# n00b001/neuro-genetic-pong-self-play

Measured on AMD Instinct MI355X. Metric: env-steps/sec (GA evaluation loop, self-play) + generations/sec at pop=65536 per GPU, higher is better.
Workload: dtype f32 hidden + certified f64 argmax; genomes f64

## Files before the change

neuro-genetic-pong-self-play_amd/csrc/pg_cascade.hpp:

```cpp
#pragma once

#include <hip/hip_runtime.h>
#include <stdint.h>

#include "pg_device.hpp"
#include "pg_eval.hpp"
#include "pg_f64math.h"

namespace pg {

#ifndef PG_SLOW_INLINE
#define PG_SLOW_INLINE __forceinline__
#endif
#ifndef PG_LOAD_BATCH
#define PG_LOAD_BATCH 2
#endif
#ifndef PG_RES_WAVES
#define PG_RES_WAVES 0
#endif
#if PG_RES_WAVES > 0
#define PG_RES_BOUNDS __launch_bounds__(256, PG_RES_WAVES)
#else
#define PG_RES_BOUNDS __launch_bounds__(256)
#endif
// ... 234 lines not shown
  n.e = v[D + P * O * 2 + O];
  n.ct = make_cert(n.e);
}

template <int U, int O>
__device__ __forceinline__ void load_rec(NetP<U, O> &n, const float *__restrict__ r) {
  constexpr int P = NetP<U, O>::P;
  constexpr int F = rec_floats<U, O>();
  const float4 *s = reinterpret_cast<const float4 *>(r);
  float v[F];
#pragma unroll
  for (int q = 0; q < F / 4; ++q) {
    const float4 x = s[q];
    v[4 * q] = x.x;
    v[4 * q + 1] = x.y;
    v[4 * q + 2] = x.z;
    v[4 * q + 3] = x.w;
  }
#pragma unroll
  for (int p = 0; p < P; ++p)
#pragma unroll
    for (int i = 0; i < 7; ++i) n.w1[p][i] = float2v{v[(p * 7 + i) * 2], v[(p * 7 + i) * 2 + 1]};
#pragma unroll
  for (int p = 0; p < P; ++p)
#pragma unroll
    for (int o = 0; o < O; ++o) n.w2[p][o] = float2v{v[P * 14 + (p * O + o) * 2], v[P * 14 + (p * O + o) * 2 + 1]};
#pragma unroll
  for (int o = 0; o < O; ++o) n.c[o] = v[P * 14 + P * O * 2 + o];
  n.e = v[P * 14 + P * O * 2 + O];
  n.ct = make_cert(n.e);
}

template <int U, int O, bool kBiasIn = false>
__device__ __forceinline__ void partial_pk(const NetP<U, O> &n, const int k[6], float acc[O]) {
  constexpr int P = NetP<U, O>::P;
  float2v kx[6];
#pragma unroll
  for (int i = 0; i < 6; ++i) {
    const float f = (float)k[i];
    kx[i] = float2v{f, f};
  }
  float2v a2[O];
#pragma unroll
  for (int o = 0; o < O; ++o) a2[o] = kBiasIn ? float2v{n.c[o], n.c[o]} : float2v{0.f, 0.f};
#pragma unroll
  for (int p = 0; p < P; p += 2) {
    constexpr int kStep = 2;
    const bool two = p + 1 < P;
    float2v a = n.w1[p][6], b = two ? n.w1[p + 1][6] : float2v{0.f, 0.f};
#pragma unroll
    for (int i = 0; i < 6; ++i) {
      a = __builtin_elementwise_fma(n.w1[p][i], kx[i], a);
      if (two) b = __builtin_elementwise_fma(n.w1[p + 1][i], kx[i], b);
    }
    const float2v qa = float2v{__builtin_amdgcn_exp2f(a.x), __builtin_amdgcn_exp2f(a.y)} + 1.0f;
    const float2v qb = float2v{__builtin_amdgcn_exp2f(b.x), __builtin_amdgcn_exp2f(b.y)} + 1.0f;
    const float2v sa = float2v{__builtin_amdgcn_rcpf(qa.x), __builtin_amdgcn_rcpf(qa.y)};
    const float2v sb = float2v{__builtin_amdgcn_rcpf(qb.x), __builtin_amdgcn_rcpf(qb.y)};
#pragma unroll
    for (int o = 0; o < O; ++o) {
      a2[o] = __builtin_elementwise_fma(n.w2[p][o], sa, a2[o]);
      if (two) a2[o] = __builtin_elementwise_fma(n.w2[p + 1][o], sb, a2[o]);
    }
    (void)kStep;
  }
#pragma unroll
  for (int o = 0; o < O; ++o) acc[o] = a2[o].x + a2[o].y;
}

template <int HL, int U, int O>
__device__ __forceinline__ float frame_bound_wave(const float *__restrict__ rec, const int k[6], int lane64) {
  constexpr int P = NetP<U, O>::P;
  constexpr int F = rec_floats<U, O>();
  constexpr float kOR = (float)out_roundings<HL, U>();
  float acc[O];
#pragma unroll
  for (int o = 0; o < O; ++o) acc[o] = 0.f;
#pragma unroll 1
  for (int t = lane64; t < HL * 2 * P; t += 64) {
    const int hl = t % HL, u = t / HL, p = u >> 1, h = u & 1;
    const float *r = rec + hl * F;
    float w[7];
#pragma unroll
    for (int i = 0; i < 7; ++i) w[i] = r[(p * 7 + i) * 2 + h];
    float w2[O];
#pragma unroll
    for (int o = 0; o < O; ++o) w2[o] = r[P * 14 + (p * O + o) * 2 + h];
    float a = w[6], rr = fabsf(w[6]), ws = fabsf(w[6]);
#pragma unroll
    for (int i = 0; i < 6; ++i) {
      a = fmaf(w[i], (float)k[i], a);
      rr = fmaf(fabsf(w[i]), (float)k[i], rr);
      ws += fabsf(w[i]);
    }
    const float da = (rr + ws * (320.f * 9.5367431640625e-7f)) * (11.f * kU);
    const float sl = fminf(0.25f, __builtin_amdgcn_exp2f(2.f * da - fabsf(a)));
    const float s = __builtin_amdgcn_rcpf(__builtin_amdgcn_exp2f(a) + 1.0f);
    const float ds = sl * da * 0.6931471805599453f + s * ((5.f + kOR) * kU) + 7.8886090522101181e-31f;
#pragma unroll
    for (int o = 0; o < O; ++o) acc[o] = fmaf(fabsf(w2[o]), ds, acc[o]);
// ... 28 lines not shown
      top1 = gt ? z[o] : top1;
    }
  }
  const float tw = __builtin_amdgcn_exp2f(__builtin_fmaf(top1, 1.4426950408889634f, c.ee));
  const int uns_res = (top1 - top2 > c.e2 + tw && top1 > c.lowz) ? w : -1;
  return top1 >= c.tlo ? sat_res : uns_res;
}

template <int O>
__device__ __forceinline__ int certify_c8(const float z[O], const Cert &c) {
  if constexpr (O == 3) {
    const float top1 = fmaxf(fmaxf(z[0], z[1]), z[2]);
    const float top2 = __builtin_amdgcn_fmed3f(z[0], z[1], z[2]);
    const int wc = z[0] == top1 ? -6 : (z[1] == top1 ? 6 : 0);
    const float tw = __builtin_amdgcn_exp2f(__builtin_fmaf(top1, 1.4426950408889634f, c.ee));
#ifndef PG_CERT_FULL_SAT
    const bool ok = ((top2 < c.tlo) & (top1 > c.thi)) | ((top1 < c.tlo) & (top1 - top2 > c.e2 + tw) & (top1 > c.lowz));
    return ok ? wc : -1;
#else
    const bool m0 = z[0] >= c.tlo, m1 = z[1] >= c.tlo;
    const int fc = m0 ? -6 : (m1 ? 6 : 0);
    const float zf = m0 ? z[0] : (m1 ? z[1] : z[2]);
    const int sat_res = zf > c.thi ? fc : -1;
    const int uns_res = (top1 - top2 > c.e2 + tw && top1 > c.lowz) ? wc : -1;
    return top1 >= c.tlo ? sat_res : uns_res;
#endif
  } else {
    const int idx = certify_c<O>(z, c);
    return idx < 0 ? -1 : index_to_move(idx);
  }
}

template <int O>
__device__ __forceinline__ int tight_gap_move(const float z[O], float e, const Cert &c) {
  float top1, top2;
  int w;
  if constexpr (O == 3) {
    top1 = fmaxf(fmaxf(z[0], z[1]), z[2]);
    top2 = __builtin_amdgcn_fmed3f(z[0], z[1], z[2]);
    w = z[0] == top1 ? 0 : (z[1] == top1 ? 1 : 2);
  } else {
    top1 = z[0];
    top2 = -3.0e38f;
    w = 0;
#pragma unroll
    for (int o = 1; o < O; ++o) {
      const bool gt = z[o] > top1;
      top2 = gt ? top1 : fmaxf(top2, z[o]);
      w = gt ? o : w;
      top1 = gt ? z[o] : top1;
    }
  }
  const float tw = __builtin_amdgcn_exp2f(__builtin_fmaf(top1, 1.4426950408889634f, -51.985645f)) +
                   4.4408921e-16f;
  const bool ok = (top2 - e >= 22.2f) & (top1 < c.tlo) & (top1 - top2 > (2.f * e + tw) * 1.000001f);
  return ok ? index_to_move(w) : -1;
}

template <int O>
__device__ __forceinline__ int certify(const float z[O], float e) {
  constexpr float kTlo = 36.7367f, kThi = 36.7369f;
  constexpr float kLowZ = -708.0f;
  const float tlo = kTlo - e, thi = kThi + e;
  int sat_res = z[O - 1] > thi ? O - 1 : -1;
#pragma unroll
  for (int o = O - 2; o >= 0; --o) sat_res = z[o] > thi ? o : (z[o] >= tlo ? -1 : sat_res);
// ... 405 lines not shown
```

neuro-genetic-pong-self-play_amd/csrc/pg_device.hpp:

```cpp
#pragma once

#include <hip/hip_runtime.h>
#include <stdint.h>

#include "pg_f64math.h"

namespace pg {

#define PG_ANY(c) __builtin_expect(__builtin_amdgcn_ballot_w64(c) != 0, 0)

constexpr int kFieldW = 160;
constexpr int kFieldH = 160;
constexpr int kPaddleH = 16;
constexpr int kPaddleW = 4;
constexpr int kLeftPaddleX = 16;
constexpr int kRightPaddleX = 140;
constexpr int kBallH = 4;
constexpr int kBallW = 2;
constexpr int kPaddleYMin = -8;
constexpr int kPaddleYMax = 152;
constexpr int kPaddleSpeed = 3;
constexpr int kCpuSpeed = 2;
constexpr int kServeDelay = 30;
constexpr int kBallVx0 = 2;
// ... 152 lines not shown
  k = (k << 8) | (uint64_t)((s.rpy + 8) & 255);
  k = (k << 2) | (uint64_t)(act_r & 3);
  k = (k << 2) | (uint64_t)(act_l & 3);
  return k;
}
#ifndef PG_RALLY_START
#define PG_RALLY_START 256
#endif
#ifndef PG_RALLY_STRIDE
#define PG_RALLY_STRIDE 4
#endif
constexpr int kRallyStart = PG_RALLY_START;
constexpr int kRallyStride = PG_RALLY_STRIDE;
#ifndef PG_RALLY_SPAN0
#define PG_RALLY_SPAN0 64
#endif
constexpr int kRallyHits = 8;
static_assert(kRallyHits <= 8, "rally_key caps hits at 8");
constexpr int kRallySpan0 = PG_RALLY_SPAN0;

__device__ inline int paddle_c2(int py) {
  const int lo = py < 0 ? 0 : py;
  const int hi = py + kPaddleH - 1 > kFieldH - 1 ? kFieldH - 1 : py + kPaddleH - 1;
  return lo + hi;
}

__device__ inline int clamp_action(int c2, int code) {
  return c2 < 32 ? 2 : (c2 > 2 * (kFieldH - 16) ? 1 : code);
}
__device__ inline int clamp_move(int c2, int move) {
  static_assert(kPaddleSpeed == 3, "doubled moves of 6");
  return c2 < 32 ? 6 : (c2 > 2 * (kFieldH - 16) ? -6 : move);
}
__device__ inline int move_code(int move) { return move < 0 ? 1 : (move > 0 ? 2 : 0); }

__device__ inline int hardcoded(int by2, int me2) { return by2 < me2 ? 1 : (by2 > me2 ? 2 : 0); }
__device__ inline int hardcoded_move(int by2, int me2) { return by2 < me2 ? -6 : (by2 > me2 ? 6 : 0); }

__device__ inline int index_to_code(int idx) {
  return (int)__builtin_amdgcn_ubfe(9u, 2u * (unsigned)idx, 2u);
}
__device__ inline int index_to_move(int idx) {
  return (int)__builtin_amdgcn_sbfe(0x0006FA, 8u * (unsigned)idx, 8u);
}

struct PongK {
  int bx2, by2, vx2, vy2, vis, timer, dir, hits, point, lc2, rc2, s1, s2, one_player;
  uint64_t seed;
  static_assert(kBallH == 4 && kPaddleH == 16 && kBallW == 2, "the doubled-unit constants below");
  static constexpr int kC2Reset = 2 * 72 + kPaddleH - 1;

  __device__ void reset(uint64_t s, int one_p) {
    bx2 = 2 * 79 + kBallW - 1; by2 = 2 * 78 + kBallH - 1; vx2 = 0; vy2 = 0; vis = 0; timer = kServeDelay;
    dir = 1; hits = 0; point = 0; lc2 = kC2Reset; rc2 = kC2Reset; s1 = 0; s2 = 0; one_player = one_p; seed = s;
  }
  __device__ bool done() const { return s1 >= kDoneScore || s2 >= kDoneScore; }

  __device__ static int c2_clip(int c2) { return paddle_c2((c2 - (kPaddleH - 1)) >> 1); }
  __device__ static int drift2(int c2, int h) {
    const int down = c2 <= 31 ? min((37 - c2) / 6, h) : 0;
    const int up = c2 >= 289 ? min((c2 - 283) / 6, h) : 0;
    return c2 + 2 * kPaddleSpeed * (down - up);
  }

  template <class ServeOf>
  __device__ int step(int right_move, int left_move, ServeOf serve_of, bool any_one_player) {
    int ev = kStepFly;
    rc2 += right_move;
    int nl = lc2 + left_move;
    if (__builtin_expect(any_one_player, 0)) {
      const int cpu_dy = vis ? ((by2 < lc2 - 4) ? -1 : ((by2 > lc2 + 4) ? 1 : 0)) : 0;
      const int moved = lc2 + 2 * kCpuSpeed * cpu_dy;
      constexpr int lo = 2 * kPaddleYMin + kPaddleH - 1, hi = 2 * kPaddleYMax + kPaddleH - 1;
      nl = one_player ? (moved < lo ? lo : (moved > hi ? hi : moved)) : nl;
    }
    lc2 = nl;

    constexpr int top2 = kBallH - 1;
    constexpr int bot2 = 2 * (kFieldH - kBallH) + kBallH - 1;
    constexpr int lface = kLeftPaddleX + kPaddleW, rface = kRightPaddleX;
    constexpr int left2 = 2 * (lface - 1) + kBallW - 1;
    constexpr int right2 = 2 * (rface - kBallW + 1) + kBallW - 1;
    const bool play = vis != 0;
    const int nx2 = bx2 + vx2;
    int ny2 = by2 + vy2;
    const bool wall_top = ny2 < top2, wall_bot = ny2 > bot2;
    ny2 = wall_top ? 2 * top2 - ny2 : (wall_bot ? 2 * bot2 - ny2 : ny2);
    vy2 = (wall_top || wall_bot) ? -vy2 : vy2;
    const bool to_left = play && nx2 <= left2;
    const bool to_right = play && nx2 >= right2;
    bx2 = nx2;
    by2 = ny2;
    if (PG_ANY(to_left || to_right || !play)) {
    if (to_left || to_right) {
      const int d = ny2 - (to_left ? lc2 : rc2);
      if (d >= -18 && d <= 18) {
        hits += 1;
        const int mag = min(kBallVx0 + (hits >> 2), kBallVxMax);
        const int q = (abs(d) * 43) >> 8;
        bx2 = to_left ? 2 * lface + kBallW - 1 : 2 * (rface - kBallW) + kBallW - 1;
        vx2 = to_left ? 2 * mag : -2 * mag;
        vy2 = d < 0 ? -2 * q : 2 * q;
        ev = hits >= kRallyHits ? kStepRally : kStepBounce;
      } else {
        s2 += to_left ? 1 : 0;
        s1 += to_right ? 1 : 0;
        dir = to_left ? -1 : 1;
        timer = kServeDelay;
        vis = 0;
        ev = kStepPoint;
      }
    }
    if (!play) {
      timer = timer > 0 ? timer - 1 : 0;
      if (timer == 0 && !done()) {
        const uint32_t e = serve_of(point);
        bx2 = 2 * 79 + kBallW - 1;
        by2 = 2 * (int)(e & 255u) + kBallH - 1;
        vy2 = 2 * ((int)(e >> 8) - 2);
        vx2 = 2 * dir * kBallVx0;
        hits = 0;
        vis = 1;
        point += 1;
      }
    }
    }
    return ev;
  }

  __device__ uint64_t key(int act_r, int act_l) const {
    Pong s;
    s.bx = (bx2 - (kBallW - 1)) >> 1;
    s.by = (by2 - (kBallH - 1)) >> 1;
    s.vx = vx2 >> 1;
    s.vy = vy2 >> 1;
    s.vis = vis;
    s.timer = timer;
    s.dir = dir;
    s.hits = hits;
    s.point = point;
    s.lpy = (lc2 - (kPaddleH - 1)) >> 1;
    s.rpy = (rc2 - (kPaddleH - 1)) >> 1;
    return rally_key(s, act_r, act_l);
  }
};

template <int CTRL>
__device__ __forceinline__ float dpp_mov(float v) {
  return __int_as_float(__builtin_amdgcn_update_dpp(0, __float_as_int(v), CTRL, 0xF, 0xF, false));
}

template <int L>
__device__ __forceinline__ float group_sum(float v) {
  if constexpr (L >= 2) v += dpp_mov<0xB1>(v);
  if constexpr (L >= 4) v += dpp_mov<0x4E>(v);
  if constexpr (L >= 8) v += dpp_mov<0x141>(v);
  if constexpr (L >= 16) v += dpp_mov<0x140>(v);
  if constexpr (L >= 32) {
    const auto r = __builtin_amdgcn_permlane16_swap(__float_as_uint(v), __float_as_uint(v), false, false);
    v = __uint_as_float(r[0]) + __uint_as_float(r[1]);
  }
  if constexpr (L >= 64) {
    const auto r = __builtin_amdgcn_permlane32_swap(__float_as_uint(v), __float_as_uint(v), false, false);
    v = __uint_as_float(r[0]) + __uint_as_float(r[1]);
  }
  return v;
}

template <int L>
__device__ __forceinline__ float group_max(float v) {
  if constexpr (L >= 2) v = fmaxf(v, dpp_mov<0xB1>(v));
  if constexpr (L >= 4) v = fmaxf(v, dpp_mov<0x4E>(v));
  if constexpr (L >= 8) v = fmaxf(v, dpp_mov<0x141>(v));
  if constexpr (L >= 16) v = fmaxf(v, dpp_mov<0x140>(v));
  if constexpr (L >= 32) v = fmaxf(v, __shfl_xor(v, 16, 64));
// ... 126 lines not shown
```

neuro-genetic-pong-self-play_amd/csrc/pg_service.hpp:

```cpp
#pragma once

#include <hip/hip_runtime.h>

#include "../../include/pong_ga.h"
#include "pg_cascade.hpp"
#include "pg_device.hpp"
#include "pg_eval.hpp"
#include "pg_f64math.h"

namespace pg {

#ifndef PG_SVC_PRIO
#define PG_SVC_PRIO 3
#endif
#ifndef PG_SVC_BATCH
#define PG_SVC_BATCH 1
#endif

#ifndef PG_INLINE_SVC
#define PG_INLINE_SVC 1
#endif
#ifndef PG_INLINE_PRIO
#define PG_INLINE_PRIO 3
#endif
// ... 244 lines not shown
                         d, 0, k[q]);
              }
              d |= 256;
            } else {
              d |= 512;
            }
            if (lane64 == 0) {
              slots[sl[q]].idx = d;
              __threadfence_block();
              lds_st(&slots[sl[q]].flag, 2);
            }
          }
        }
      }
    }
    return;
  }

  const int lig = threadIdx.x & (L - 1);
  const int side = lig >= HL ? 1 : 0;
  const int hl = lig & (HL - 1);
  const int leader = lane64 & ~(L - 1);
  const int wave_slot0 = __builtin_amdgcn_readfirstlane((int)(threadIdx.x >> 6)) * (64 / L) * 2;
  const auto slot_grp = [&]() { return wave_slot0 + (fresh_lane64() / L) * 2; };
  const auto slot_me = [&]() {
    const int l = fresh_lane64();
    return wave_slot0 + (l / L) * 2 + ((l & (L - 1)) >= HL ? 1 : 0);
  };
  const WT *genomes = (const WT *)p.genomes;
  const WT *opponents = (const WT *)p.opponents;

  NetP<U, O> net;
  PongK st;
  int kind = 0, act_r = 0, act_l = 0, total = 0, fstart = 0, tend = 0, c_vis = 0, tab_off = 0;
  int sframe = 0;
#ifndef PG_NO_HIDDEN_JUMP
  constexpr bool kVisByFrames = kUntraced && !kHorizon;
#else
  constexpr bool kVisByFrames = false;
#endif
  const WT *gm = genomes;
  uint32_t slow = 0, c_fwd = 0, c_steps = 0, c_games = 0, fails = 0, plateau = 0, inwave = 0, skipped = 0, hidden = 0;

  const int games_total = active_total(p);
  int w;
  {
    int ww = 0;
    if (lig == 0) ww = (int)atomicAdd(p.work, 1u);
    w = group_broadcast<L>(ww, leader);
  }
  bool fresh = true;
  bool live = w < games_total;
  const auto park = [&]() {
    st.bx2 = 2 * 79 + kBallW - 1;
    st.by2 = 2 * 78 + kBallH - 1;
    st.vx2 = st.vy2 = 0;
    st.vis = 2;
    st.one_player = 0;
    kind = kOppNN;
    tend = 0x7fffffff;
    fstart = 0x3fffffff;
    fresh = false;
  };
  if (kInline && !live) park();
  int w_scripted = 1, w_onep = 1;
  int top = 1;
#ifdef PG_PROBE_EXTRA
  float probe_v = 0.f;
  float2v probe_p = float2v{0.f, 0.f};
  int probe_s = 0;
#endif
#ifdef PG_START_PROBE
  uint64_t probe_fresh = 0;
  const uint64_t probe_t0 = __builtin_amdgcn_s_memtime();
#endif
#ifdef PG_SERVE_STAGES
  uint64_t st_acc[24];
#pragma unroll
  for (int i = 0; i < 24; ++i) st_acc[i] = 0;
#endif
#ifdef PG_DECIDE_PROBE
  uint64_t probe_dec = 0;
  const uint64_t probe_t0 = __builtin_amdgcn_s_memtime();
#endif
#ifdef PG_TIMELINE
  uint64_t t_start = 0;
  uint32_t g_fails = 0, g_slow = 0;
#endif
#ifdef PG_PATH_PROBE
  uint32_t pp_frames = 0, pp_rally = 0, pp_face = 0, pp_fail = 0, pp_hidden = 0;
#define PG_PP(cnt, cond) \
  if (__builtin_amdgcn_ballot_w64(cond) != 0) cnt += 1
#else
#define PG_PP(cnt, cond)
#endif
  if (kInline ? __builtin_amdgcn_ballot_w64(live) != 0 : live) for (;;) {
#ifdef PG_START_PROBE
    const bool any_fresh = __builtin_amdgcn_ballot_w64(fresh) != 0;
    const uint64_t probe_f0 = __builtin_amdgcn_s_memtime();
#endif
    PG_PP(pp_frames, true);
    sframe += 1;
#ifdef PG_TIMELINE
    constexpr bool kJumps = !kHorizon;
#else
    const bool kJumps = !kHorizon && (kUntraced || p.trace == nullptr);
#endif
    if (top) {
    if (fresh) {
      const int i = w / p.n_games;
      const int g = w - i * p.n_games;
      kind = p.kind[w];
      const WT *gr = genomes + (long)genome_row(p, i) * p.gstride;
      const bool nn = side && kind == kOppNN && p.n_opponents > 0;
      const int oj = nn ? min(max(p.opp[w], 0), p.n_opponents - 1) : 0;
      gm = nn ? opponents + (long)oj * p.ostride : gr;
      const int rec = nn ? p.n_genomes + oj : i;
      load_rec<U, O>(net, p.recs + ((long)rec * HL + hl) * rec_floats<U, O>());
      const int sx = slot_me();
      if (kInline && hl == 0) slots[sx].rec = rec;
#pragma unroll
      for (int o = 0; o < O; ++o) net.c[o] = hl == 0 ? 0.5f * net.c[o] : 0.f;
      st.reset(0, kind == kOppRomCpu);
      if (kHorizon || !tabbed) st.seed = game_seed(p.seed, g);
      tab_off = g * kServeTabPoints;
      act_r = act_l = total = 0;
      c_vis = kVisByFrames ? sframe - 1 : 0;
      fstart = sframe - 1;
      tend = sframe + p.timeout_thresh;
      fresh = false;
      if (hl == 0) slots[sx].n_memo = 0;
      if (lig == 0) slots[sx].rally_at = -1;
      if (kHorizon && lig == 0) {
        const int gx = threadIdx.x / L;
        hz[gx].sum = 0.0;
        hz[gx].eps = hz[gx].s1 = hz[gx].s2 = hz[gx].zd = 0;
      }
#ifdef PG_TIMELINE
      t_start = wall_clock64();
      g_fails = g_slow = 0;
#endif
    }
#ifdef PG_START_PROBE
    if (any_fresh) probe_fresh += __builtin_amdgcn_s_memtime() - probe_f0;
#endif
#ifndef PG_NO_HIDDEN_JUMP
    {
      const bool hid = !st.vis && st.timer >= 2;
      PG_PP(pp_hidden, hid);
      if (kJumps && hid) {
        const int h = st.timer - 1;
        st.rc2 = PongK::drift2(st.rc2, h);
        if (!st.one_player) st.lc2 = PongK::drift2(st.lc2, h);
        st.timer = 1;
        act_r = clamp_move(st.rc2, 0);
        act_l = clamp_move(st.lc2, 0);
        fstart -= h;
        tend -= h;
        hidden += h;
      }
    }
#endif
    w_scripted = __builtin_amdgcn_readfirstlane(__builtin_amdgcn_ballot_w64(kind != kOppNN) != 0);
    w_onep = __builtin_amdgcn_readfirstlane(__builtin_amdgcn_ballot_w64(st.one_player != 0) != 0);
    top = 0;
    }
    const int pvis = st.vis, pbx2 = st.bx2, pby2 = st.by2;
#ifdef PG_PATH_PROBE
    const int pt_b = st.point, hits_b = st.hits;
#endif
    const int ev = st.step(act_r, act_l, [&](int pt) {
      return tabbed && pt < kServeTabPoints ? serve_tab[tab_off + pt] : Pong::serve_entry(st.seed, pt);
    }, w_onep != 0);
    PG_PP(pp_face, ev != kStepFly || st.hits != hits_b || st.point != pt_b);
    const int vis = st.vis;
    const int bx2 = st.bx2, by2 = st.by2;
    const int rc2 = st.rc2;
    int lc2 = st.lc2;
    if (__builtin_expect(w_onep, 0)) lc2 = PongK::c2_clip(st.lc2);
    int left, right;
    {
      const int lbx2 = pvis ? pbx2 : bx2, lby2 = pvis ? pby2 : by2;
      const int k[6] = {bx2, by2, lbx2, lby2, rc2, lc2};
      float acc[O], z[O];
      partial_pk<U, O, true>(net, k, acc);
#pragma unroll
      for (int o = 0; o < O; ++o) z[o] = group_sum<HL>(acc[o]);
      int code = certify_c8<O>(z, net.ct);
#ifdef PG_PROBE_EXTRA
      pg_probe_extra<PG_PROBE_EXTRA>(net.w1[0][0], net.w1[1][1], z[0], z[1], probe_v, probe_p, probe_s);
#endif
      const bool left_nn = kind == kOppNN;
      if (side && !left_nn) code = 0;
      if (vis != 1) code = 0;
#ifdef PG_ABLATE_SLOW
      if (code == -1) code = z[1] > z[0] ? 6 : -6;
#endif
      PG_PP(pp_fail, code == -1);
      if (PG_ANY(code == -1)) {
      if (code == -1) {
        fails += 1;
#ifdef PG_TIMELINE
        g_fails += 1;
#endif
#ifndef PG_NO_TIGHT
        int mv = tight_gap_move<O>(z, net.e, net.ct);
        if (mv == -1)
#else
        int mv = -1;
#endif
        {
          const int idx = plateau_f32<O>(z, net.e);
          mv = idx >= 0 ? index_to_move(idx) : -1;
        }
        inwave += mv != -1 ? 1 : 0;
        code = mv;
      }
#ifdef PG_ABLATE_SERVE
      if (code == -1) code = z[1] > z[0] ? 6 : -6;
#endif
      if (kInline && PG_ANY(code == -1)) {
        uint64_t key = 0;
        int nm = 0;
        const int sx = slot_me();
        if (code == -1) {
          key = memo_key(k);
          nm = slots[sx].n_memo;
          int hit = -1;
#pragma unroll 1
          for (int c = 0; c < kMemo && c < nm; ++c)
            if (slots[sx].memo_key[c] == key) hit = slots[sx].memo_idx[c];
          code = hit;
        }
        const int kn[6] = {side ? 320 - bx2 : bx2, by2, side ? 320 - lbx2 : lbx2, lby2, side ? lc2 : rc2,
                           side ? rc2 : lc2};
        const float my_e = net.e;
        uint64_t need = __builtin_amdgcn_ballot_w64(code == -1 && hl == 0);
        if (need) {
#ifdef PG_DECIDE_PROBE
        const uint64_t probe_d0 = __builtin_amdgcn_s_memtime();
#endif
        if constexpr (PG_INLINE_PRIO > 0) __builtin_amdgcn_s_setprio(PG_INLINE_PRIO);
#pragma unroll 1
        do {
          const int src = (int)__builtin_ctzll(need);
          need &= need - 1;
          InlineReq r;
#pragma unroll
          for (int i = 0; i < 6; ++i) r.k[i] = __builtin_amdgcn_readlane(kn[i], src);
#pragma unroll
          for (int i = 0; i < 6; ++i) r.kr[i] = __builtin_amdgcn_readlane(k[i], src);
          r.rec = p.recs + (long)__builtin_amdgcn_readlane(slots[sx].rec, src) * HL * rec_floats<U, O>();
#pragma unroll
          for (int o = O; o < 4; ++o) r.z[o] = 0.f;
#pragma unroll
          for (int o = 0; o < O; ++o) r.z[o] = __int_as_float(__builtin_amdgcn_readlane(__float_as_int(z[o]), src));
          r.e = __int_as_float(__builtin_amdgcn_readlane(__float_as_int(my_e), src));
          const uint64_t ga = (uint64_t)gm;
          const WT *g = (const WT *)(((uint64_t)__builtin_amdgcn_readlane((int)(ga >> 32), src) << 32) |
                                     (uint32_t)__builtin_amdgcn_readlane((int)(uint32_t)ga, src));
#if defined(PG_SERVE_TWICE)
          serve_inline<U, HL, O, WT>(p, g, r, lds_svc + wave * f64_lds_doubles(H, O), lane64, st_acc);
          const int ans = serve_inline<U, HL, O, WT>(p, g, r, lds_svc + wave * f64_lds_doubles(H, O), lane64, st_acc + 12);
#elif defined(PG_SERVE_STAGES)
          const int ans = serve_inline<U, HL, O, WT>(p, g, r, lds_svc + wave * f64_lds_doubles(H, O), lane64, st_acc);
#else
          const int ans = serve_inline<U, HL, O, WT>(p, g, r, lds_svc + wave * f64_lds_doubles(H, O), lane64);
#endif
          if ((lane64 & ~(HL - 1)) == src) {
            slow += (ans >> 8) & 1;
            plateau += (ans >> 9) & 1;
            inwave += ans >> 10;
            code = index_to_move(ans & 255);
            if (hl == 0) {
              const int c = nm % kMemo;
              slots[sx].memo_key[c] = key;
              slots[sx].memo_idx[c] = code;
              slots[sx].n_memo = nm + 1;
            }
          }
        } while (need);
        if constexpr (PG_INLINE_PRIO > 0) __builtin_amdgcn_s_setprio(0);
        {
#if defined(PG_RELOAD_ALL)
          load_rec<U, O>(net, p.recs + ((long)slots[sx].rec * HL + hl) * rec_floats<U, O>());
#elif !defined(PG_NO_RELOAD)
          load_rec_out<U, O>(net, p.recs + ((long)slots[sx].rec * HL + hl) * rec_floats<U, O>());
#endif
#ifndef PG_NO_RELOAD
#pragma unroll
          for (int o = 0; o < O; ++o) net.c[o] = hl == 0 ? 0.5f * net.c[o] : 0.f;
#endif
#ifdef PG_SERVE_STAGES
          {
            const uint64_t r0 = __builtin_amdgcn_s_memtime();
            asm volatile("s_waitcnt vmcnt(0) lgkmcnt(0)" ::: "memory");
            st_acc[5] += __builtin_amdgcn_s_memtime() - r0;
            st_acc[11] += 1;
          }
#endif
#ifdef PG_DECIDE_PROBE
          asm volatile("s_waitcnt vmcnt(0)" ::: "memory");
          probe_dec += __builtin_amdgcn_s_memtime() - probe_d0;
#endif
        }
        }
      }
      if (!kInline && PG_ANY(code == -1) && code == -1) {
        const int sx = slot_me();
        const uint64_t key = memo_key(k);
        const int nm = slots[sx].n_memo;
        int hit = -1;
#pragma unroll 1
        for (int c = 0; c < kMemo && c < nm; ++c)
          if (slots[sx].memo_key[c] == key) hit = slots[sx].memo_idx[c];
        if (hit != -1) {
          code = hit;
        } else {
          if (hl == 0) {
            const int kn[6] = {side ? 320 - bx2 : bx2, by2, side ? 320 - lbx2 : lbx2, lby2, side ? lc2 : rc2,
                               side ? rc2 : lc2};
            slots[sx].g = gm;
#pragma unroll
            for (int i = 0; i < 6; ++i) slots[sx].k[i] = kn[i];
#pragma unroll
            for (int o = 0; o < O; ++o) slots[sx].z[o] = z[o];
            slots[sx].e = net.e;
            __threadfence_block();
            lds_st(&slots[sx].flag, 1);
            __hip_atomic_fetch_add(&posted, 1, __ATOMIC_RELAXED, __HIP_MEMORY_SCOPE_WORKGROUP);
          }
          while (lds_ld(&slots[sx].flag) != 2) __builtin_amdgcn_s_sleep(1);
          __threadfence_block();
          const int ans = slots[sx].idx;
          slow += (ans >> 8) & 1;
#ifdef PG_TIMELINE
          g_slow += 1;
#endif
          plateau += ans >> 9;
          code = index_to_move(ans & 255);
          if (hl == 0) {
            const int c = nm % kMemo;
            slots[sx].memo_key[c] = key;
            slots[sx].memo_idx[c] = code;
            slots[sx].n_memo = nm + 1;
            lds_st(&slots[sx].flag, 0);
          }
        }
      }
      }
      const int mine = code;
      const int other = other_half<L>(mine);
      right = side ? other : mine;
      left = side ? mine : other;
      if (__builtin_expect(w_scripted, 0) && !left_nn) {
        left = vis ? hardcoded_move(by2, lc2) : 0;
        if (kind == kOppScore && st.s1 > st.s2) left = 0;
      }
      if constexpr (!kVisByFrames) c_vis += vis;
    }
    act_l = clamp_move(lc2, left);
    act_r = clamp_move(rc2, right);
#ifndef PG_TIMELINE
    if (!kUntraced && p.trace) {
      const int frames = sframe - fstart;
      if (w < p.trace_games && frames <= p.trace_cap && lig == 0 && (!kInline || live))
        p.trace[(long)w * p.trace_cap + frames - 1] = (uint8_t)(move_code(act_r) | (move_code(act_l) << 2) | (vis << 4));
    }
#endif
    const bool same = ev != kStepPoint;
#ifndef PG_NO_RALLY_SKIP
#ifdef PG_TIMELINE
    constexpr bool kTracing = false;
#else
    const bool kTracing = !kUntraced && p.trace != nullptr;
#endif
    const bool rally_check = !kTracing && !kHorizon && ev == kStepRally;
#else
    constexpr bool rally_check = false;
#endif
    PG_PP(pp_rally, rally_check);
    bool over = sframe > tend;
    if constexpr (kHorizon) over = over || sframe - fstart >= p.horizon;
    if (PG_ANY((kHorizon ? !same : ev >= kStepPoint) || over)) {
    if (!same) {
      total += sframe - 1 - (tend - p.timeout_thresh);
      tend = sframe + p.timeout_thresh;
      over = st.s1 >= p.win_score || st.s2 >= p.win_score || st.done();
      if constexpr (kHorizon) over = over || sframe - fstart >= p.horizon;
      if (lig == 0) slots[slot_grp()].rally_at = -1;
    }
#ifndef PG_NO_RALLY_SKIP
    const int timeout = sframe - (tend - p.timeout_thresh);
    if (rally_check && timeout <= p.timeout_thresh) {
      const int rs = slot_grp();
      const uint64_t key = st.key(move_code(act_r), move_code(act_l));
      const int at = slots[rs].rally_at;
      if (at > timeout || at < 0) {
        if (lig == 0) {
          slots[rs].rally_key = key;
          slots[rs].rally_at = timeout;
          slots[rs].rally_span = kRallySpan0;
        }
      } else if (slots[rs].rally_key == key) {
        const int rest = p.timeout_thresh + 1 - timeout;
        fstart -= rest;
        skipped += rest;
        tend = sframe - 1;
      } else if (timeout - at >= slots[rs].rally_span) {
        if (lig == 0) {
          slots[rs].rally_key = key;
          slots[rs].rally_at = timeout;
          slots[rs].rally_span = 2 * slots[rs].rally_span;
        }
      }
    }
    over = over || sframe > tend;
// ... 41 lines not shown
        uint32_t *tl = (uint32_t *)(p.trace + (long)w * p.trace_cap);
        tl[0] = (uint32_t)t_start;
        tl[1] = (uint32_t)wall_clock64();
        tl[2] = g_fails;
        tl[3] = g_slow;
        if (p.trace_cap >= 24) {
          tl[4] = blockIdx.x;
          tl[5] = (uint32_t)wave;
        }
      }
#endif
      c_steps += sframe - fstart;
      const int vis_frames = kVisByFrames ? sframe - c_vis - (st.s1 + st.s2) : c_vis;
      c_fwd += (kind == kOppNN ? 2u : 1u) * (uint32_t)vis_frames;
      c_games += 1;
      int ww = 0;
      if (lig == 0) ww = (int)atomicAdd(p.work, 1u);
      w = group_broadcast<L>(ww, leader);
      if constexpr (kInline) {
        if (w >= games_total) {
          live = false;
          park();
        } else {
          fresh = true;
        }
      } else {
        if (w >= games_total) break;
        fresh = true;
      }
    }
    if constexpr (kInline) {
      if (__builtin_amdgcn_ballot_w64(live) == 0) break;
    }
    top = __builtin_amdgcn_readfirstlane(__builtin_amdgcn_ballot_w64(fresh || (kJumps && !st.vis && st.timer >= 2)) != 0);
    }
  }
  if (p.counters && c_games) {
    if (lig == 0) {
      atomicAdd((unsigned long long *)&p.counters[0], (unsigned long long)(c_steps - skipped - hidden));
      if (hidden) atomicAdd((unsigned long long *)&p.counters[12], (unsigned long long)hidden);
      atomicAdd((unsigned long long *)&p.counters[1], (unsigned long long)c_fwd);
      atomicAdd((unsigned long long *)&p.counters[3], (unsigned long long)c_games);
      if (skipped) atomicAdd((unsigned long long *)&p.counters[8], (unsigned long long)skipped);
    }
    if (hl == 0 && slow) atomicAdd((unsigned long long *)&p.counters[2], (unsigned long long)slow);
    if (hl == 0 && fails) atomicAdd((unsigned long long *)&p.counters[4], (unsigned long long)fails);
    if (hl == 0 && plateau) atomicAdd((unsigned long long *)&p.counters[5], (unsigned long long)plateau);
    if (hl == 0 && inwave) atomicAdd((unsigned long long *)&p.counters[6], (unsigned long long)inwave);
  }
#ifdef PG_DECIDE_PROBE
  if (p.counters && lane64 == 0) {
    atomicAdd((unsigned long long *)&p.counters[13], (unsigned long long)probe_dec);
    atomicAdd((unsigned long long *)&p.counters[14], (unsigned long long)(__builtin_amdgcn_s_memtime() - probe_t0));
    atomicAdd((unsigned long long *)&p.counters[15], 1ull);
  }
#endif
#ifdef PG_START_PROBE
  if (p.counters && lane64 == 0) {
    atomicAdd((unsigned long long *)&p.counters[13], (unsigned long long)probe_fresh);
    atomicAdd((unsigned long long *)&p.counters[14], (unsigned long long)(__builtin_amdgcn_s_memtime() - probe_t0));
    atomicAdd((unsigned long long *)&p.counters[15], 1ull);
  }
#endif
#ifdef PG_PATH_PROBE
  if (p.counters && lane64 == 0) {
    atomicAdd((unsigned long long *)&p.counters[11], (unsigned long long)pp_frames);
    atomicAdd((unsigned long long *)&p.counters[10], (unsigned long long)pp_rally);
    atomicAdd((unsigned long long *)&p.counters[13], (unsigned long long)pp_face);
    atomicAdd((unsigned long long *)&p.counters[14], (unsigned long long)pp_fail);
    atomicAdd((unsigned long long *)&p.counters[15], (unsigned long long)pp_hidden);
  }
#endif
#ifdef PG_PROBE_EXTRA
  if (p.counters && probe_v == 1234.5f && probe_p.x == 1234.5f && probe_s == 1234567) p.counters[15] = 1;
#endif
#ifdef PG_SERVE_STAGES
  if (p.hard_log && lane64 == 0)
#pragma unroll
    for (int i = 0; i < 24; ++i)
      if (st_acc[i]) atomicAdd((unsigned long long *)&((uint64_t *)p.hard_log)[i], (unsigned long long)st_acc[i]);
#endif
  if (lane64 == 0) atomicAdd(&waves_done, 1);
}

inline size_t service_records_bytes(int n_genomes, int n_opponents, int L, int U, int O) {
  const int F = ((U + 1) / 2 * 2 * (7 + O) + O + 1 + 3) / 4 * 4;
  return ((size_t)n_genomes + (size_t)(n_opponents > 0 ? n_opponents : 0)) * (size_t)(L / 2) * F * sizeof(float);
}

template <int L, int U, int O, typename WT, bool kSplitTrace = false>
inline int32_t launch_service(const EvalParams &p, hipStream_t s) {
  constexpr int kSvcThreads = svc_threads<U>();
  const bool inl = p.horizon > 0 ? inline_service<L, U, true>() : inline_service<L, U, false>();
  const int GPB = (kSvcThreads / 64 - (inl ? 0 : 1)) * (64 / L);
  const size_t lds = (size_t)f64_lds_doubles(p.nodes[1], O) * sizeof(double) * (inl ? kSvcThreads / 64 : 1);
  const int want = (p.total + GPB - 1) / GPB;
  const int cap = num_cus() * 2;
  const int grid = want < cap ? want : cap;
  if (grid <= 0) return PG_OK;
  if (!p.recs) return fail(PG_ERR_INVALID, "split kernel: no lane-record workspace");
  if (!kSplitTrace && p.horizon > 0)
// ... 31 lines not shown
```

Baseline: 13.14 billion.

## Keep Pong state in float and fold masking into certification to shorten step path

Converts the per-lane Pong state (ball, velocity, paddle centres) to floats so network inputs feed straight into the packed FMA without int-to-float conversions. Moves are encoded as unit floats scaled by FMA. A precomputed move mask is merged into certification. The step collapses wall and face checks into two fabs comparisons behind one wave-uniform branch, stores the event in state, and puts the rally/point bookkeeping behind a ballot. This shortens the common flying-ball frame at the cost of float-int casts on rare paths and added state registers.

```diff
diff --git a/neuro-genetic-pong-self-play_amd/csrc/pg_cascade.hpp b/neuro-genetic-pong-self-play_amd/csrc/pg_cascade.hpp
--- a/neuro-genetic-pong-self-play_amd/csrc/pg_cascade.hpp
+++ b/neuro-genetic-pong-self-play_amd/csrc/pg_cascade.hpp
@@ -290,14 +290,11 @@
 }
 
 template <int U, int O, bool kBiasIn = false>
-__device__ __forceinline__ void partial_pk(const NetP<U, O> &n, const int k[6], float acc[O]) {
+__device__ __forceinline__ void partial_pk(const NetP<U, O> &n, const float kf[6], float acc[O]) {
   constexpr int P = NetP<U, O>::P;
   float2v kx[6];
 #pragma unroll
-  for (int i = 0; i < 6; ++i) {
-    const float f = (float)k[i];
-    kx[i] = float2v{f, f};
-  }
+  for (int i = 0; i < 6; ++i) kx[i] = float2v{kf[i], kf[i]};
   float2v a2[O];
 #pragma unroll
   for (int o = 0; o < O; ++o) a2[o] = kBiasIn ? float2v{n.c[o], n.c[o]} : float2v{0.f, 0.f};
@@ -324,6 +321,13 @@
   }
 #pragma unroll
   for (int o = 0; o < O; ++o) acc[o] = a2[o].x + a2[o].y;
+}
+template <int U, int O, bool kBiasIn = false>
+__device__ __forceinline__ void partial_pk(const NetP<U, O> &n, const int k[6], float acc[O]) {
+  float kf[6];
+#pragma unroll
+  for (int i = 0; i < 6; ++i) kf[i] = (float)k[i];
+  partial_pk<U, O, kBiasIn>(n, kf, acc);
 }
 
 template <int HL, int U, int O>
@@ -418,6 +422,26 @@
 }
 
 template <int O>
+__device__ __forceinline__ float certify_c8m(const float z[O], const Cert &c, float m, bool &failed) {
+#ifndef PG_CERT_FULL_SAT
+  if constexpr (O == 3) {
+    const float top1 = fmaxf(fmaxf(z[0], z[1]), z[2]);
+    const float top2 = __builtin_amdgcn_fmed3f(z[0], z[1], z[2]);
+    const float wc = z[0] == top1 ? -m : (z[1] == top1 ? m : 0.f);
+    const float tw = __builtin_amdgcn_exp2f(__builtin_fmaf(top1, 1.4426950408889634f, c.ee));
+    const bool ok = ((top2 < c.tlo) & (top1 > c.thi)) | ((top1 < c.tlo) & (top1 - top2 > c.e2 + tw) & (top1 > c.lowz));
+    failed = !ok & (m != 0.f);
+    return wc;
+  } else
+#endif
+  {
+    const int mv = certify_c8<O>(z, c);
+    failed = mv == -1 && m != 0.f;
+    return m * move_f(mv);
+  }
+}
+
+template <int O>
 __device__ __forceinline__ int tight_gap_move(const float z[O], float e, const Cert &c) {
   float top1, top2;
   int w;
diff --git a/neuro-genetic-pong-self-play_amd/csrc/pg_device.hpp b/neuro-genetic-pong-self-play_amd/csrc/pg_device.hpp
--- a/neuro-genetic-pong-self-play_amd/csrc/pg_device.hpp
+++ b/neuro-genetic-pong-self-play_amd/csrc/pg_device.hpp
@@ -208,10 +208,18 @@
   static_assert(kPaddleSpeed == 3, "doubled moves of 6");
   return c2 < 32 ? 6 : (c2 > 2 * (kFieldH - 16) ? -6 : move);
 }
+constexpr float kMoveStep = 2 * kPaddleSpeed;
+constexpr float kUndecided = 2.f;
+__device__ inline float clamp_move(float c2, float move) {
+  return c2 < 32.f ? 1.f : (c2 > (float)(2 * (kFieldH - 16)) ? -1.f : move);
+}
+__device__ inline float move_f(int mv) { return mv == -1 ? kUndecided : (float)(mv / (2 * kPaddleSpeed)); }
 __device__ inline int move_code(int move) { return move < 0 ? 1 : (move > 0 ? 2 : 0); }
+__device__ inline int move_code(float move) { return move < 0.f ? 1 : (move > 0.f ? 2 : 0); }
 
 __device__ inline int hardcoded(int by2, int me2) { return by2 < me2 ? 1 : (by2 > me2 ? 2 : 0); }
 __device__ inline int hardcoded_move(int by2, int me2) { return by2 < me2 ? -6 : (by2 > me2 ? 6 : 0); }
+__device__ inline float hardcoded_move(float by2, float me2) { return by2 < me2 ? -1.f : (by2 > me2 ? 1.f : 0.f); }
 
 __device__ inline int index_to_code(int idx) {
   return (int)__builtin_amdgcn_ubfe(9u, 2u * (unsigned)idx, 2u);
@@ -221,14 +229,21 @@
 }
 
 struct PongK {
-  int bx2, by2, vx2, vy2, vis, timer, dir, hits, point, lc2, rc2, s1, s2, one_player;
+  float bx2, by2, vx2, vy2, lbx2, lby2, lc2, rc2;
+  int vis, timer, dir, hits, point, s1, s2, one_player, ev;
   uint64_t seed;
+#ifdef PG_PATH_PROBE
+  uint32_t pp_block = 0;
+#endif
   static_assert(kBallH == 4 && kPaddleH == 16 && kBallW == 2, "the doubled-unit constants below");
   static constexpr int kC2Reset = 2 * 72 + kPaddleH - 1;
+  static constexpr float kHiddenX = 1048576.f;
 
   __device__ void reset(uint64_t s, int one_p) {
-    bx2 = 2 * 79 + kBallW - 1; by2 = 2 * 78 + kBallH - 1; vx2 = 0; vy2 = 0; vis = 0; timer = kServeDelay;
+    bx2 = kHiddenX; by2 = 2 * 78 + kBallH - 1; vx2 = 0.f; vy2 = 0.f; vis = 0; timer = kServeDelay;
+    lbx2 = bx2; lby2 = by2;
     dir = 1; hits = 0; point = 0; lc2 = kC2Reset; rc2 = kC2Reset; s1 = 0; s2 = 0; one_player = one_p; seed = s;
+    ev = kStepFly;
   }
   __device__ bool done() const { return s1 >= kDoneScore || s2 >= kDoneScore; }
 
@@ -239,15 +254,15 @@
     return c2 + 2 * kPaddleSpeed * (down - up);
   }
 
-  template <class ServeOf>
-  __device__ int step(int right_move, int left_move, ServeOf serve_of, bool any_one_player) {
-    int ev = kStepFly;
-    rc2 += right_move;
-    int nl = lc2 + left_move;
+  template <class ServeOf, class AfterEvent>
+  __device__ void step(float right_move, float left_move, ServeOf serve_of, bool any_one_player,
+                       AfterEvent after_event) {
+    rc2 = __builtin_fmaf(right_move, kMoveStep, rc2);
+    float nl = __builtin_fmaf(left_move, kMoveStep, lc2);
     if (__builtin_expect(any_one_player, 0)) {
-      const int cpu_dy = vis ? ((by2 < lc2 - 4) ? -1 : ((by2 > lc2 + 4) ? 1 : 0)) : 0;
-      const int moved = lc2 + 2 * kCpuSpeed * cpu_dy;
-      constexpr int lo = 2 * kPaddleYMin + kPaddleH - 1, hi = 2 * kPaddleYMax + kPaddleH - 1;
+      const float cpu_dy = vis ? ((by2 < lc2 - 4.f) ? -1.f : ((by2 > lc2 + 4.f) ? 1.f : 0.f)) : 0.f;
+      const float moved = lc2 + (float)(2 * kCpuSpeed) * cpu_dy;
+      constexpr float lo = 2 * kPaddleYMin + kPaddleH - 1, hi = 2 * kPaddleYMax + kPaddleH - 1;
       nl = one_player ? (moved < lo ? lo : (moved > hi ? hi : moved)) : nl;
     }
     lc2 = nl;
@@ -257,26 +272,37 @@
     constexpr int lface = kLeftPaddleX + kPaddleW, rface = kRightPaddleX;
     constexpr int left2 = 2 * (lface - 1) + kBallW - 1;
     constexpr int right2 = 2 * (rface - kBallW + 1) + kBallW - 1;
-    const bool play = vis != 0;
-    const int nx2 = bx2 + vx2;
-    int ny2 = by2 + vy2;
-    const bool wall_top = ny2 < top2, wall_bot = ny2 > bot2;
-    ny2 = wall_top ? 2 * top2 - ny2 : (wall_bot ? 2 * bot2 - ny2 : ny2);
-    vy2 = (wall_top || wall_bot) ? -vy2 : vy2;
-    const bool to_left = play && nx2 <= left2;
-    const bool to_right = play && nx2 >= right2;
+    static_assert((left2 + right2) % 2 == 0 && (top2 + bot2) % 2 == 0, "integer mid points");
+    lbx2 = bx2;
+    lby2 = by2;
+    const float nx2 = bx2 + vx2;
+    float ny2 = by2 + vy2;
+    const bool face = !(__builtin_fabsf(nx2 - 0.5f * (left2 + right2)) < 0.5f * (right2 - left2));
+    const bool wall = __builtin_fabsf(ny2 - 0.5f * (top2 + bot2)) > 0.5f * (bot2 - top2);
     bx2 = nx2;
     by2 = ny2;
-    if (PG_ANY(to_left || to_right || !play)) {
+    if (PG_ANY(face || wall)) {
+#ifdef PG_PATH_PROBE
+    pp_block += 1;
+#endif
+    ev = kStepFly;
+    if (wall) {
+      ny2 = ny2 < (float)top2 ? 2 * top2 - ny2 : 2 * bot2 - ny2;
+      vy2 = -vy2;
+      by2 = ny2;
+    }
+    const bool play = vis != 0;
+    const bool to_left = play && nx2 <= (float)left2;
+    const bool to_right = play && nx2 >= (float)right2;
     if (to_left || to_right) {
-      const int d = ny2 - (to_left ? lc2 : rc2);
+      const int d = (int)(ny2 - (to_left ? lc2 : rc2));
       if (d >= -18 && d <= 18) {
         hits += 1;
         const int mag = min(kBallVx0 + (hits >> 2), kBallVxMax);
         const int q = (abs(d) * 43) >> 8;
         bx2 = to_left ? 2 * lface + kBallW - 1 : 2 * (rface - kBallW) + kBallW - 1;
-        vx2 = to_left ? 2 * mag : -2 * mag;
-        vy2 = d < 0 ? -2 * q : 2 * q;
+        vx2 = (float)(to_left ? 2 * mag : -2 * mag);
+        vy2 = (float)(d < 0 ? -2 * q : 2 * q);
         ev = hits >= kRallyHits ? kStepRally : kStepBounce;
       } else {
         s2 += to_left ? 1 : 0;
@@ -284,6 +310,7 @@
         dir = to_left ? -1 : 1;
         timer = kServeDelay;
         vis = 0;
+        bx2 = kHiddenX;
         ev = kStepPoint;
       }
     }
@@ -292,31 +319,33 @@
       if (timer == 0 && !done()) {
         const uint32_t e = serve_of(point);
         bx2 = 2 * 79 + kBallW - 1;
-        by2 = 2 * (int)(e & 255u) + kBallH - 1;
-        vy2 = 2 * ((int)(e >> 8) - 2);
-        vx2 = 2 * dir * kBallVx0;
+        by2 = (float)(2 * (int)(e & 255u) + kBallH - 1);
+        vy2 = (float)(2 * ((int)(e >> 8) - 2));
+        vx2 = (float)(2 * dir * kBallVx0);
+        lbx2 = bx2;
+        lby2 = by2;
         hits = 0;
         vis = 1;
         point += 1;
       }
     }
-    }
-    return ev;
+    after_event();
+    }
   }
 
   __device__ uint64_t key(int act_r, int act_l) const {
     Pong s;
-    s.bx = (bx2 - (kBallW - 1)) >> 1;
-    s.by = (by2 - (kBallH - 1)) >> 1;
-    s.vx = vx2 >> 1;
-    s.vy = vy2 >> 1;
+    s.bx = ((int)bx2 - (kBallW - 1)) >> 1;
+    s.by = ((int)by2 - (kBallH - 1)) >> 1;
+    s.vx = (int)vx2 >> 1;
+    s.vy = (int)vy2 >> 1;
     s.vis = vis;
     s.timer = timer;
     s.dir = dir;
     s.hits = hits;
     s.point = point;
-    s.lpy = (lc2 - (kPaddleH - 1)) >> 1;
-    s.rpy = (rc2 - (kPaddleH - 1)) >> 1;
+    s.lpy = ((int)lc2 - (kPaddleH - 1)) >> 1;
+    s.rpy = ((int)rc2 - (kPaddleH - 1)) >> 1;
     return rally_key(s, act_r, act_l);
   }
 };
diff --git a/neuro-genetic-pong-self-play_amd/csrc/pg_service.hpp b/neuro-genetic-pong-self-play_amd/csrc/pg_service.hpp
--- a/neuro-genetic-pong-self-play_amd/csrc/pg_service.hpp
+++ b/neuro-genetic-pong-self-play_amd/csrc/pg_service.hpp
@@ -300,7 +300,8 @@
 
   NetP<U, O> net;
   PongK st;
-  int kind = 0, act_r = 0, act_l = 0, total = 0, fstart = 0, tend = 0, c_vis = 0, tab_off = 0;
+  int kind = 0, total = 0, fstart = 0, tend = 0, c_vis = 0, tab_off = 0;
+  float act_r = 0.f, act_l = 0.f;
   int sframe = 0;
 #ifndef PG_NO_HIDDEN_JUMP
   constexpr bool kVisByFrames = kUntraced && !kHorizon;
@@ -320,10 +321,11 @@
   bool fresh = true;
   bool live = w < games_total;
   const auto park = [&]() {
-    st.bx2 = 2 * 79 + kBallW - 1;
-    st.by2 = 2 * 78 + kBallH - 1;
-    st.vx2 = st.vy2 = 0;
+    st.bx2 = st.lbx2 = 2 * 79 + kBallW - 1;
+    st.by2 = st.lby2 = 2 * 78 + kBallH - 1;
+    st.vx2 = st.vy2 = 0.f;
     st.vis = 2;
+    st.ev = kStepFly;
     st.one_player = 0;
     kind = kOppNN;
     tend = 0x7fffffff;
@@ -332,7 +334,9 @@
   };
   if (kInline && !live) park();
   int w_scripted = 1, w_onep = 1;
+  float m_move = 0.f;
   int top = 1;
+  const auto remask = [&]() { m_move = ((side && kind != kOppNN) || st.vis != 1) ? 0.f : 1.f; };
 #ifdef PG_PROBE_EXTRA
   float probe_v = 0.f;
   float2v probe_p = float2v{0.f, 0.f};
@@ -356,7 +360,7 @@
   uint32_t g_fails = 0, g_slow = 0;
 #endif
 #ifdef PG_PATH_PROBE
-  uint32_t pp_frames = 0, pp_rally = 0, pp_face = 0, pp_fail = 0, pp_hidden = 0;
+  uint32_t pp_frames = 0, pp_rally = 0, pp_fail = 0, pp_hidden = 0;
 #define PG_PP(cnt, cond) \
   if (__builtin_amdgcn_ballot_w64(cond) != 0) cnt += 1
 #else
@@ -418,11 +422,11 @@
       PG_PP(pp_hidden, hid);
       if (kJumps && hid) {
         const int h = st.timer - 1;
-        st.rc2 = PongK::drift2(st.rc2, h);
-        if (!st.one_player) st.lc2 = PongK::drift2(st.lc2, h);
+        st.rc2 = (float)PongK::drift2((int)st.rc2, h);
+        if (!st.one_player) st.lc2 = (float)PongK::drift2((int)st.lc2, h);
         st.timer = 1;
-        act_r = clamp_move(st.rc2, 0);
-        act_l = clamp_move(st.lc2, 0);
+        act_r = clamp_move(st.rc2, 0.f);
+        act_l = clamp_move(st.lc2, 0.f);
         fstart -= h;
         tend -= h;
         hidden += h;
@@ -431,42 +435,39 @@
 #endif
     w_scripted = __builtin_amdgcn_readfirstlane(__builtin_amdgcn_ballot_w64(kind != kOppNN) != 0);
     w_onep = __builtin_amdgcn_readfirstlane(__builtin_amdgcn_ballot_w64(st.one_player != 0) != 0);
+    remask();
     top = 0;
     }
-    const int pvis = st.vis, pbx2 = st.bx2, pby2 = st.by2;
-#ifdef PG_PATH_PROBE
-    const int pt_b = st.point, hits_b = st.hits;
-#endif
-    const int ev = st.step(act_r, act_l, [&](int pt) {
+    st.step(act_r, act_l, [&](int pt) {
       return tabbed && pt < kServeTabPoints ? serve_tab[tab_off + pt] : Pong::serve_entry(st.seed, pt);
-    }, w_onep != 0);
-    PG_PP(pp_face, ev != kStepFly || st.hits != hits_b || st.point != pt_b);
+    }, w_onep != 0, [&]() {
+      remask();
+    });
     const int vis = st.vis;
-    const int bx2 = st.bx2, by2 = st.by2;
-    const int rc2 = st.rc2;
-    int lc2 = st.lc2;
-    if (__builtin_expect(w_onep, 0)) lc2 = PongK::c2_clip(st.lc2);
-    int left, right;
+    const float bx2 = st.bx2, by2 = st.by2, lbx2 = st.lbx2, lby2 = st.lby2;
+    const float rc2 = st.rc2;
+    float lc2 = st.lc2;
+    if (__builtin_expect(w_onep, 0)) lc2 = (float)PongK::c2_clip((int)st.lc2);
+    float left, right;
     {
-      const int lbx2 = pvis ? pbx2 : bx2, lby2 = pvis ? pby2 : by2;
-      const int k[6] = {bx2, by2, lbx2, lby2, rc2, lc2};
+      const float kf[6] = {bx2, by2, lbx2, lby2, rc2, lc2};
       float acc[O], z[O];
-      partial_pk<U, O, true>(net, k, acc);
+      partial_pk<U, O, true>(net, kf, acc);
 #pragma unroll
       for (int o = 0; o < O; ++o) z[o] = group_sum<HL>(acc[o]);
-      int code = certify_c8<O>(z, net.ct);
+      bool failed;
+      float code = certify_c8m<O>(z, net.ct, m_move, failed);
 #ifdef PG_PROBE_EXTRA
       pg_probe_extra<PG_PROBE_EXTRA>(net.w1[0][0], net.w1[1][1], z[0], z[1], probe_v, probe_p, probe_s);
 #endif
-      const bool left_nn = kind == kOppNN;
-      if (side && !left_nn) code = 0;
-      if (vis != 1) code = 0;
 #ifdef PG_ABLATE_SLOW
-      if (code == -1) code = z[1] > z[0] ? 6 : -6;
-#endif
-      PG_PP(pp_fail, code == -1);
-      if (PG_ANY(code == -1)) {
-      if (code == -1) {
+      if (failed) code = z[1] > z[0] ? 1.f : -1.f;
+      failed = false;
+#endif
+      PG_PP(pp_fail, failed);
+      if (PG_ANY(failed)) {
+      if (failed) code = kUndecided;
+      if (code == kUndecided) {
         fails += 1;
 #ifdef PG_TIMELINE
         g_fails += 1;
@@ -482,28 +483,29 @@
           mv = idx >= 0 ? index_to_move(idx) : -1;
         }
         inwave += mv != -1 ? 1 : 0;
-        code = mv;
+        code = move_f(mv);
       }
 #ifdef PG_ABLATE_SERVE
-      if (code == -1) code = z[1] > z[0] ? 6 : -6;
-#endif
-      if (kInline && PG_ANY(code == -1)) {
+      if (code == kUndecided) code = z[1] > z[0] ? 1.f : -1.f;
+#endif
+      if (kInline && PG_ANY(code == kUndecided)) {
+        const int k[6] = {(int)bx2, (int)by2, (int)lbx2, (int)lby2, (int)rc2, (int)lc2};
         uint64_t key = 0;
         int nm = 0;
         const int sx = slot_me();
-        if (code == -1) {
+        if (code == kUndecided) {
           key = memo_key(k);
           nm = slots[sx].n_memo;
           int hit = -1;
 #pragma unroll 1
           for (int c = 0; c < kMemo && c < nm; ++c)
             if (slots[sx].memo_key[c] == key) hit = slots[sx].memo_idx[c];
-          code = hit;
-        }
-        const int kn[6] = {side ? 320 - bx2 : bx2, by2, side ? 320 - lbx2 : lbx2, lby2, side ? lc2 : rc2,
-                           side ? rc2 : lc2};
+          code = move_f(hit);
+        }
+        const int kn[6] = {side ? 320 - k[0] : k[0], k[1], side ? 320 - k[2] : k[2], k[3], side ? k[5] : k[4],
+                           side ? k[4] : k[5]};
         const float my_e = net.e;
-        uint64_t need = __builtin_amdgcn_ballot_w64(code == -1 && hl == 0);
+        uint64_t need = __builtin_amdgcn_ballot_w64(code == kUndecided && hl == 0);
         if (need) {
 #ifdef PG_DECIDE_PROBE
         const uint64_t probe_d0 = __builtin_amdgcn_s_memtime();
@@ -517,7 +519,8 @@
 #pragma unroll
           for (int i = 0; i < 6; ++i) r.k[i] = __builtin_amdgcn_readlane(kn[i], src);
 #pragma unroll
-          for (int i = 0; i < 6; ++i) r.kr[i] = __builtin_amdgcn_readlane(k[i], src);
+          for (int i = 0; i < 6; ++i)
+            r.kr[i] = (int)__int_as_float(__builtin_amdgcn_readlane(__float_as_int(kf[i]), src));
           r.rec = p.recs + (long)__builtin_amdgcn_readlane(slots[sx].rec, src) * HL * rec_floats<U, O>();
 #pragma unroll
           for (int o = O; o < 4; ++o) r.z[o] = 0.f;
@@ -539,11 +542,12 @@
             slow += (ans >> 8) & 1;
             plateau += (ans >> 9) & 1;
             inwave += ans >> 10;
-            code = index_to_move(ans & 255);
+            const int mv = index_to_move(ans & 255);
+            code = move_f(mv);
             if (hl == 0) {
               const int c = nm % kMemo;
               slots[sx].memo_key[c] = key;
-              slots[sx].memo_idx[c] = code;
+              slots[sx].memo_idx[c] = mv;
               slots[sx].n_memo = nm + 1;
             }
           }
@@ -574,7 +578,8 @@
         }
         }
       }
-      if (!kInline && PG_ANY(code == -1) && code == -1) {
+      if (!kInline && PG_ANY(code == kUndecided) && code == kUndecided) {
+        const int k[6] = {(int)bx2, (int)by2, (int)lbx2, (int)lby2, (int)rc2, (int)lc2};
         const int sx = slot_me();
         const uint64_t key = memo_key(k);
         const int nm = slots[sx].n_memo;
@@ -583,11 +588,11 @@
         for (int c = 0; c < kMemo && c < nm; ++c)
           if (slots[sx].memo_key[c] == key) hit = slots[sx].memo_idx[c];
         if (hit != -1) {
-          code = hit;
+          code = move_f(hit);
         } else {
           if (hl == 0) {
-            const int kn[6] = {side ? 320 - bx2 : bx2, by2, side ? 320 - lbx2 : lbx2, lby2, side ? lc2 : rc2,
-                               side ? rc2 : lc2};
+            const int kn[6] = {side ? 320 - k[0] : k[0], k[1], side ? 320 - k[2] : k[2], k[3], side ? k[5] : k[4],
+                               side ? k[4] : k[5]};
             slots[sx].g = gm;
 #pragma unroll
             for (int i = 0; i < 6; ++i) slots[sx].k[i] = kn[i];
@@ -606,29 +611,31 @@
           g_slow += 1;
 #endif
           plateau += ans >> 9;
-          code = index_to_move(ans & 255);
+          const int mv = index_to_move(ans & 255);
+          code = move_f(mv);
           if (hl == 0) {
             const int c = nm % kMemo;
             slots[sx].memo_key[c] = key;
-            slots[sx].memo_idx[c] = code;
+            slots[sx].memo_idx[c] = mv;
             slots[sx].n_memo = nm + 1;
             lds_st(&slots[sx].flag, 0);
           }
         }
       }
       }
-      const int mine = code;
-      const int other = other_half<L>(mine);
+      const float mine = clamp_move(side ? lc2 : rc2, code);
+      const float other = __int_as_float(other_half<L>(__float_as_int(mine)));
       right = side ? other : mine;
       left = side ? mine : other;
-      if (__builtin_expect(w_scripted, 0) && !left_nn) {
-        left = vis ? hardcoded_move(by2, lc2) : 0;
-        if (kind == kOppScore && st.s1 > st.s2) left = 0;
+      if (__builtin_expect(w_scripted, 0) && kind != kOppNN) {
+        left = vis ? hardcoded_move(by2, lc2) : 0.f;
+        if (kind == kOppScore && st.s1 > st.s2) left = 0.f;
+        left = clamp_move(lc2, left);
       }
       if constexpr (!kVisByFrames) c_vis += vis;
     }
-    act_l = clamp_move(lc2, left);
-    act_r = clamp_move(rc2, right);
+    act_l = left;
+    act_r = right;
 #ifndef PG_TIMELINE
     if (!kUntraced && p.trace) {
       const int frames = sframe - fstart;
@@ -636,6 +643,11 @@
         p.trace[(long)w * p.trace_cap + frames - 1] = (uint8_t)(move_code(act_r) | (move_code(act_l) << 2) | (vis << 4));
     }
 #endif
+    bool over0 = sframe > tend;
+    if constexpr (kHorizon) over0 = over0 || sframe - fstart >= p.horizon;
+    if (PG_ANY((kHorizon ? st.ev == kStepPoint : st.ev >= kStepPoint) || over0)) {
+    const int ev = st.ev;
+    st.ev = kStepFly;
     const bool same = ev != kStepPoint;
 #ifndef PG_NO_RALLY_SKIP
 #ifdef PG_TIMELINE
@@ -650,7 +662,6 @@
     PG_PP(pp_rally, rally_check);
     bool over = sframe > tend;
     if constexpr (kHorizon) over = over || sframe - fstart >= p.horizon;
-    if (PG_ANY((kHorizon ? !same : ev >= kStepPoint) || over)) {
     if (!same) {
       total += sframe - 1 - (tend - p.timeout_thresh);
       tend = sframe + p.timeout_thresh;
@@ -758,6 +769,7 @@
     if constexpr (kInline) {
       if (__builtin_amdgcn_ballot_w64(live) == 0) break;
     }
+    remask();
     top = __builtin_amdgcn_readfirstlane(__builtin_amdgcn_ballot_w64(fresh || (kJumps && !st.vis && st.timer >= 2)) != 0);
     }
   }
@@ -792,7 +804,7 @@
   if (p.counters && lane64 == 0) {
     atomicAdd((unsigned long long *)&p.counters[11], (unsigned long long)pp_frames);
     atomicAdd((unsigned long long *)&p.counters[10], (unsigned long long)pp_rally);
-    atomicAdd((unsigned long long *)&p.counters[13], (unsigned long long)pp_face);
+    atomicAdd((unsigned long long *)&p.counters[13], (unsigned long long)st.pp_block);
     atomicAdd((unsigned long long *)&p.counters[14], (unsigned long long)pp_fail);
     atomicAdd((unsigned long long *)&p.counters[15], (unsigned long long)pp_hidden);
   }
```

Result: faster. 13.88 billion (median of 6 runs) (+5.6%).
